# martende/findex

Hardware: AMD Instinct MI355X
Metric: rank_queries_per_sec (higher is better)
Workload: dtype u64

## Files before the change

### findex_amd/csrc/fmx_search4.h

```cpp
#pragma once
#include <type_traits>
#include "fmx_device.h"
#include "fmx_pool_deal.h"

namespace fmx {

constexpr int kSThreads = 256;

__device__ __forceinline__ uint32_t fetch4(const uint8_t *__restrict__ pat, uint64_t pos) {
  if (pos >= 4) {
    uint32_t d;
    __builtin_memcpy(&d, pat + pos - 4, 4);
    return __builtin_bswap32(d);
  }
  uint32_t r = 0;
  for (uint32_t j = 0; j < (uint32_t)pos; j++) r |= (uint32_t)pat[pos - 1 - j] << (8 * j);
  return r;
}


__device__ __forceinline__ uint32_t pat_chunk(const uint8_t *__restrict__ pat, const uint64_t *__restrict__ own,
                                              uint64_t end, uint32_t len, uint32_t j) {
  const uint32_t have = len > 4u * j ? len - 4u * j : 0u;
  const uint64_t pos = end - 4ull * j;
// ... 32 lines not shown
#ifdef FMX_SEARCHLOG
  const unsigned long long sl_t0 = __builtin_amdgcn_s_memrealtime();
  unsigned long long sl_t1 = 0, sl_look = 0, sl_draw = 0;
  uint32_t sl_claim = 0, sl_last = 0;
  uint32_t sl_batches = 0, sl_claims = 0;
#endif
  if (threadIdx.x == 0 && blockIdx.x < kCensusBlocks) {
    counters[(size_t)kCounterSlots * kCounterStride + 2u * blockIdx.x] = __builtin_amdgcn_s_memrealtime();
    if (blockIdx.x == 0) counters[(size_t)kCounterSlots * kCounterStride + 2u * kCensusBlocks] = gridDim.x;
  }
  if (spin & 0xFFFFu) {
    const unsigned long long c0 = __builtin_amdgcn_s_memrealtime();
    while (__builtin_amdgcn_s_memrealtime() - c0 < (spin & 0xFFFFu)) __builtin_amdgcn_s_sleep(32);
  }
  const uint32_t wave = (blockIdx.x * kSThreads + threadIdx.x) >> 6;
  const uint32_t nwaves = gridDim.x * (kSThreads / 64);
  const uint32_t grp = (threadIdx.x & 63) / G;
  auto load_off_raw = [&](uint64_t bt, uint64_t &v0, uint64_t &v1) {
    const uint64_t pid = bt * P + grp;
    const uint64_t *p = po.at(pid < k ? pid : (uint64_t)k - 1);
    v0 = p[0];
    v1 = p[1];
  };
  static_assert(kSThreads == 256, "one thread per symbol fills the tables in LDS");
  __shared__ uint4 s_tab[256];
  __shared__ uint8_t s_dense[KT ? 256 : 4];
  __shared__ uint16_t s_slot[KT ? 256 : 4];
  uint64_t raw0a, raw0b, raw1a, raw1b;
  {
    const uint4 sym = ix.symtab()[threadIdx.x];
    uint8_t dn = 0;
    uint16_t sl = 0;
    if (KT) { dn = kdense[threadIdx.x]; sl = ix.slot[threadIdx.x]; }
    load_off_raw(wave, raw0a, raw0b);
    load_off_raw((uint64_t)wave + nwaves, raw1a, raw1b);
    if (KT) { s_dense[threadIdx.x] = dn; s_slot[threadIdx.x] = sl; }
    s_tab[threadIdx.x] = sym;
  }
  __syncthreads();
  const LaneConst lc = lane_const<G2 ? 4 : G>();
  const uint32_t t = G2 ? (threadIdx.x & 1u) : lc.t;
  const uint32_t lane_off = t * 16;
  uint32_t steps = 0, reqs = 0;
  struct Blk { uint4 a, b; };
  auto blk_load = [&](uint64_t vb, uint32_t b1, uint32_t upto) -> Blk {
    const uint64_t at = vb + lane_off + (uint64_t)b1 * kBlockBytes;
    Blk w;
    w.a = load_line16(at);
    w.b = make_uint4(0, 0, 0, 0);
    if constexpr (G2) {
      if (upto >= 192u) w.b = load_line16(at + 32);
    }
    return w;
  };
  auto blk_rank = [&](const Blk &w, uint32_t m1) -> uint64_t {
    if constexpr (G2) return rank_finish_g2<WIDE>(Blk2{w.a, w.b}, m1, t);
    else return rank_finish<WIDE>(w.a, m1, lc);
  };
  auto blk_bit = [&](const Blk &w, uint32_t m1) -> uint32_t {
    if constexpr (G2) return payload_bit_g2(Blk2{w.a, w.b}, m1, t);
    else return payload_bit(w.a, m1, lc);
  };
  constexpr uint32_t RB = 1u;
  auto gbc0 = [&](uint32_t v) -> uint32_t { if constexpr (G2) return pair_bcast<0>(v); else return group_bcast<G, 0>(v); };
  auto gbc1 = [&](uint32_t v) -> uint32_t { if constexpr (G2) return pair_bcast<1>(v); else return group_bcast<G, 1>(v); };
  const uint32_t nbatch = (k + P - 1) / P;
  constexpr bool kPool = G2 || RW != 0u;
  const uint32_t tix_area = kPool ? (spin >> 16) & 0xFFu : 0u;
  const bool miss_none = JT != 0u && (spin >> 31) != 0u;
  uint32_t nstatic = nbatch;
  if (tix_area) {
    const uint32_t rounds = nbatch / nwaves, held = (spin >> 24) & 0xFu;
    if (rounds >= held + 2u) nstatic = (rounds - held) * nwaves;
  }
  constexpr bool kStage = LAYOUT != kLayoutBytes;
  constexpr uint32_t kStageBytes = G2 ? 2048 : 1024, kStagePad = 16;
  __shared__ __attribute__((aligned(16))) uint32_t s_pat[kSThreads / 64][2][kStage ? (kStagePad + kStageBytes + 16) / 4 : 4];
  uint32_t par = 0;
  constexpr bool kFold = (JT && RW == 0u) || RW != 0u;
  constexpr uint32_t kParkCap = RW ? 128u : (G2 ? 96u : 64u);
  __shared__ uint64_t s_park_row[kFold ? kSThreads / 64 : 1][kFold ? kParkCap : 1];
  __shared__ uint32_t s_park_pid[kFold ? kSThreads / 64 : 1][kFold ? kParkCap : 1];
  __shared__ uint32_t s_park_it[kFold ? kSThreads / 64 : 1][kFold ? kParkCap : 1];
  uint32_t npark = 0;
  constexpr uint32_t kRowsCap = 64u + P;
  __shared__ uint64_t s_rows_row[RW ? kSThreads / 64 : 1][RW ? kRowsCap : 1];
  __shared__ uint64_t s_rows_end[RW ? kSThreads / 64 : 1][RW ? kRowsCap : 1];
  __shared__ uint32_t s_rows_pid[RW ? kSThreads / 64 : 1][RW ? kRowsCap : 1];
  __shared__ uint32_t s_rows_it[RW ? kSThreads / 64 : 1][RW ? kRowsCap : 1];
  __shared__ uint32_t s_rows_len[RW ? kSThreads / 64 : 1][RW ? kRowsCap : 1];
  uint32_t nrows = 0;
  uint32_t rsteps = 0, rlooks = 0;
  auto st_out = [](auto *p, uint64_t v) { __builtin_nontemporal_store((decltype(*p + 0))v, p); };
  auto emit = [&](uint32_t q, uint64_t a, uint64_t b) {
    if (pk_cap != ~0ull) {
      unsigned long long *pk = reinterpret_cast<unsigned long long *>(sp_out);
      const uint64_t w = b - a;
      if (w >= kPackWide) {
        const unsigned long long slot = atomicAdd(pk + k, 1ull);
        if (slot < pk_cap) { pk[(uint64_t)k + 1 + 2 * slot] = q; pk[(uint64_t)k + 2 + 2 * slot] = b; }
      }
      st_out(pk + q, a | ((w < kPackWide ? w : kPackWide) << 40));
    } else {
      st_out(sp_out + q, a);
      st_out(ep_out + q, b);
    }
  };
  const uint32_t wave_in_wg = (uint32_t)__builtin_amdgcn_readfirstlane((int)(threadIdx.x >> 6));
  const uint32_t lane64 = threadIdx.x & 63u;
  const uint64_t pat_addr = (uint64_t)(uintptr_t)pat;
  auto fix_off = [&](uint64_t bt, uint64_t v0, uint64_t v1, uint64_t &e, uint32_t &len) {
    const uint64_t pid = bt * P + grp;
    const uint64_t q = pid < k ? pid : (uint64_t)k - 1;
    const uint64_t b = po.fixed ? q * po.fixed : v0;
    e = po.fixed ? (q + 1) * po.fixed : v1;
    len = pid < k ? (uint32_t)(e - b) : 0u;
  };
  struct Stage { uint4 w; uint4 w2; uint64_t base; bool ok; };
  auto stage_issue = [&](uint64_t e, uint32_t len) {
    const uint64_t b = e - len;
    const uint64_t b0 = ((uint64_t)__builtin_amdgcn_readfirstlane((int)(uint32_t)(b >> 32)) << 32) | (uint32_t)__builtin_amdgcn_readfirstlane((int)(uint32_t)b);
    const uint64_t e1 = ((uint64_t)(uint32_t)__builtin_amdgcn_readlane((int)(uint32_t)(e >> 32), 63) << 32) | (uint32_t)__builtin_amdgcn_readlane((int)(uint32_t)e, 63);
    Stage st;
    const uint64_t al = (pat_addr + b0) & ~15ull;
    const uint64_t span = pat_addr + e1 - al;
    st.ok = kStage && span <= kStageBytes;
    st.base = al - pat_addr;
    st.w = make_uint4(0, 0, 0, 0);
    if (st.ok && 16ull * lane64 < span) st.w = load_line16(al + 16u * lane64);
    st.w2 = make_uint4(0, 0, 0, 0);
    if constexpr (G2) {
      if (st.ok && 1024ull + 16ull * lane64 < span) st.w2 = load_line16(al + 1024u + 16u * lane64);
    }
    return st;
  };
  auto stage_park = [&](const Stage &st, uint32_t area) {
    if (st.ok) *reinterpret_cast<uint4 *>(s_pat[wave_in_wg][area] + (kStagePad + 16u * lane64) / 4) = st.w;
    if constexpr (G2) {
      if (st.ok) *reinterpret_cast<uint4 *>(s_pat[wave_in_wg][area] + (kStagePad + 1024u + 16u * lane64) / 4) = st.w2;
    }
  };
  constexpr uint32_t NT = KT ? KT / 4 : 1;
  struct Tail { uint32_t c[NT]; };
  uint64_t end0, end1, raw2a, raw2b;
  uint32_t len0, len1;
  uint32_t ktl = 0, jtl = 0, r3l = 0;
  fix_off(wave, raw0a, raw0b, end0, len0);
  fix_off((uint64_t)wave + nwaves, raw1a, raw1b, end1, len1);
  Stage cur = stage_issue(end0, len0);
  stage_park(cur, par);
  Tail tail_ahead;
#pragma unroll
  for (uint32_t i = 0; i < NT; i++) tail_ahead.c[i] = (!kStage && len0 > 4u * i) ? fetch4(pat, end0 - 4ull * i) : 0u;
  auto walk_step = [&](uint32_t c, uint64_t &wsp, uint64_t &wep) {
    const uint4 en = s_tab[c];
    const uint64_t cfc = ((uint64_t)en.y << 32) | en.x;
    const uint64_t vb = ((uint64_t)en.w << 32) | en.z;
    if (vb > 1) {
      if (LAYOUT == kLayoutBytes) {
        const ByteRankReq q1 = byte_rank_issue(ix, (uint16_t)(vb - 2), wsp, lc);
        wsp = cfc + byte_rank_finish(q1, c, lc);
        wep = wsp + byte_match_bit(q1, c, lc);
      } else {
        uint32_t b1, m1;
        split448(wsp, b1, m1);
        const Blk w1 = blk_load(vb, b1, m1);
        wsp = cfc + blk_rank(w1, m1);
        wep = wsp + blk_bit(w1, m1);
      }
      reqs += R * RB;
    } else {
      const uint64_t r1 = cfc + ((vb == 1 && wsp > ix.eof) ? 1u : 0u);
      wep = cfc + ((vb == 1 && wep > ix.eof) ? 1u : 0u);
      wsp = r1;
    }
    steps++;
  };
  auto walk_parked = [&](auto last_tag) {
    constexpr bool kLast = decltype(last_tag)::value;
    while (npark) {
      const uint32_t take = npark < P ? npark : P;
      const bool actw = grp < take;
      const uint32_t slot = npark - take + (actw ? grp : 0u);
      npark -= take;
      const uint32_t wpid = actw ? s_park_pid[wave_in_wg][slot] : 0u;
      uint32_t wit = actw ? s_park_it[wave_in_wg][slot] : 0u;
      uint64_t wsp = actw ? s_park_row[wave_in_wg][slot] : 0ull;
      uint32_t wj = (uint32_t)(wsp >> 56);
      const bool wnone = wj == 0xFFu;
      const bool wkx = KX && actw && wj == 0xFEu;
      wj = (wnone || wkx) ? 0u : wj;
      wsp &= (1ull << 56) - 1;
      if constexpr (R3T && kLast) {
        while (__builtin_amdgcn_ballot_w64(actw && wj >= 3u)) {
          const bool go = actw && wj >= 3u;
          if (go) {
            wsp = r3tab[wsp] & ((1ull << 40) - 1);
            wj -= 3u;
            wit += 3u;
            steps += 3u;
          }
          r3l += (uint32_t)__builtin_popcountll(__builtin_amdgcn_ballot_w64(go && t == 0));
        }
      }
      uint64_t wep = wsp + ((actw && !wnone && !wkx) ? 1u : 0u);
      uint64_t wbegin = 0, wend = 0;
      if (actw) po.get(wpid, wbegin, wend);
      const uint32_t wlen = (uint32_t)(wend - wbegin);
      if constexpr (KX) {
        if (__builtin_amdgcn_ballot_w64(wkx)) {
          uint32_t code = 0;
#pragma unroll
          for (uint32_t j = 0; j < KT; j++) code = code * ksigma + s_dense[wkx ? pat[wend - 1 - j] : 0u];
          const uint4 xe = ktab[wkx ? code : 0u];
          if (wkx) {
            const uint64_t xsp = (((uint64_t)xe.y << 32) | xe.x) & ((1ull << 56) - 1), xep = ((uint64_t)xe.w << 32) | xe.z;
            if (xsp < xep) {
              steps += KT + 1u;
            } else {
              wsp = xsp;
              wep = xep;
              steps += xe.y >> 24;
            }
          }
          ktl += (uint32_t)__builtin_popcountll(__builtin_amdgcn_ballot_w64(wkx && t == 0));
        }
      }
      for (;;) {
        const uint32_t wrem = wlen - wit;
        if (!__builtin_amdgcn_ballot_w64(actw && wsp < wep && wrem != 0u)) break;
        const uint32_t nst = wrem < 8u ? wrem : 8u;
        uint64_t chars = 0;
        if (actw && wsp < wep) {
          if (nst == 8u) {
            uint32_t lo, hi;
            __builtin_memcpy(&lo, pat + (wend - wit - 8), 4);
            __builtin_memcpy(&hi, pat + (wend - wit - 4), 4);
            chars = ((uint64_t)__builtin_bswap32(lo) << 32) | __builtin_bswap32(hi);
          } else {
            for (uint32_t s8 = 0; s8 < nst; s8++) chars |= (uint64_t)pat[wend - wit - 1 - s8] << (8u * s8);
          }
        }
        for (uint32_t s8 = 0; s8 < 8; s8++) {
          const bool stepping = actw && wsp < wep && s8 < nst;
          if (!__builtin_amdgcn_ballot_w64(stepping)) break;
          if (stepping) walk_step((uint32_t)(chars >> (8u * s8)) & 0xFFu, wsp, wep);
        }
        wit += nst;
      }
      if (actw && t == 0) emit(wpid, wsp, wep);
    }
  };
  auto rows_phase = [&](const bool all) {
    if constexpr (RW != 0u) {
      while (nrows >= (all ? 1u : 64u)) {
        const uint32_t take = nrows < 64u ? nrows : 64u;
        const bool on = lane64 < take;
        const uint32_t slot = nrows - take + (on ? lane64 : 0u);
        nrows -= take;
        uint64_t row = on ? s_rows_row[wave_in_wg][slot] : 0ull;
        const uint64_t rend = on ? s_rows_end[wave_in_wg][slot] : 0ull;
        const uint32_t rpid = on ? s_rows_pid[wave_in_wg][slot] : 0u;
        const uint32_t rlen = on ? s_rows_len[wave_in_wg][slot] : 0u;
        uint32_t rit = on ? s_rows_it[wave_in_wg][slot] : 0u;
        bool live = on;
        while (__builtin_amdgcn_ballot_w64(live)) {
          const uint32_t rem = rlen - rit;
          bool fail = false;
          if constexpr (RW == 3u) {
            const bool tm = live && rem >= 3u;
            unsigned long long re = 0;
            uint32_t d = 0;
            if (tm) {
              re = r3tab[row];
              __builtin_memcpy(&d, pat + (rend - rit - 3), 4);
            }
            if (tm && (uint32_t)(re >> 40) == __builtin_bswap32(d << 8)) {
              rlooks++;
              row = re & ((1ull << 40) - 1);
              rit += 3;
              rsteps += 3;
            } else if (live) {
              rlooks += tm ? 1u : 0u;
              if (rem == 0u) emit(rpid, row, row + 1);
              else fail = true;
              live = false;
            }
          } else {
            const bool rm = live && rem != 0u;
            unsigned long long re = 0;
            uint32_t c = 0;
            if (rm) {
              re = r3tab[row];
              c = pat[rend - rit - 1];
            }
            const uint32_t c2 = (uint32_t)(re >> 40) & 0xFFu;
            if (rm && c == c2 && c2 != 0u) {
              rlooks++;
              row = re & ((1ull << 40) - 1);
              rit++;
              rsteps++;
            } else if (live) {
              rlooks += rm ? 1u : 0u;
              if (rem == 0u) emit(rpid, row, row + 1);
              else fail = true;
              live = false;
            }
          }
          const unsigned long long fm = __builtin_amdgcn_ballot_w64(fail);
          if (fm) {
            const uint32_t ps = npark + (uint32_t)__builtin_popcountll(fm & ((1ull << lane64) - 1ull));
            if (fail) { s_park_row[wave_in_wg][ps] = row; s_park_pid[wave_in_wg][ps] = rpid; s_park_it[wave_in_wg][ps] = rit; }
            npark += (uint32_t)__builtin_popcountll(fm);
          }
        }
      }
    }
  };
  constexpr bool kLaneWalk = !(WIDE && JT == 1u && R3T && !G2);
  auto walk_last = [&]() {
    while (npark) {
      const uint32_t take = npark < 64u ? npark : 64u;
      const bool on = lane64 < take;
      const uint32_t slot = npark - take + (on ? lane64 : 0u);
      npark -= take;
      const uint32_t wpid = on ? s_park_pid[wave_in_wg][slot] : 0u;
      const uint32_t wit0 = on ? s_park_it[wave_in_wg][slot] : 0u;
      uint64_t wsp = on ? s_park_row[wave_in_wg][slot] : 0ull;
      uint32_t wj = (uint32_t)(wsp >> 56);
      const bool wnone = wj == 0xFFu;
      const bool wkx = KX && on && wj == 0xFEu;
      wj = (wnone || wkx) ? 0u : wj;
      wsp &= (1ull << 56) - 1;
      const uint32_t n3 = R3T ? wj / 3u : 0u;
      unsigned long long word = 0;
      if constexpr (R3T) word = r3tab[n3 >= 1u ? wsp : 0ull];
      const uint64_t *own = po.at(wpid);
      const uint64_t o0 = own[0], o1 = own[1];
      const uint32_t wit = wit0 + 3u * n3;
      rsteps += 3u * n3;
      if constexpr (R3T) {
        r3l += (uint32_t)__builtin_popcountll(__builtin_amdgcn_ballot_w64(n3 >= 1u)) + (uint32_t)__builtin_popcountll(__builtin_amdgcn_ballot_w64(n3 >= 2u));
        if (n3 >= 1u) wsp = word & ((1ull << 40) - 1);
        word = r3tab[n3 >= 2u ? wsp : 0ull];
      }
      const uint64_t wbegin = po.fixed ? (uint64_t)wpid * po.fixed : o0, wend = po.fixed ? ((uint64_t)wpid + 1) * po.fixed : o1;
      const uint32_t wlen = (uint32_t)(wend - wbegin);
      const uint32_t wrem = (on && !wnone && !wkx) ? wlen - wit : 0u;
      const uint32_t nst = wrem < 8u ? wrem : 8u;
      uint64_t chars = 0;
      {
        const uint8_t *src = (nst != 0u && wlen >= 8u) ? pat + (wend - wit - nst) : reinterpret_cast<const uint8_t *>(own);
        uint32_t lo, hi;
        __builtin_memcpy(&lo, src, 4);
        __builtin_memcpy(&hi, src + 4, 4);
        const uint64_t v = ((uint64_t)__builtin_bswap32(lo) << 32) | __builtin_bswap32(hi);
        if (nst != 0u && wlen >= 8u) chars = v >> (8u * (8u - nst));
      }
      uint64_t wep = wsp;
      if constexpr (KX) {
        uint32_t code = 0;
#pragma unroll
        for (uint32_t i = 0; i < KT / 4u; i++) {
          uint32_t d;
          __builtin_memcpy(&d, wkx ? pat + (wend - 4u * (i + 1u)) : reinterpret_cast<const uint8_t *>(own), 4);
          d = __builtin_bswap32(d);
#pragma unroll
          for (uint32_t j = 0; j < 4u; j++) code = code * ksigma + s_dense[(d >> (8u * j)) & 0xFFu];
        }
        const uint4 xe = ktab[wkx ? code : 0u];
        ktl += (uint32_t)__builtin_popcountll(__builtin_amdgcn_ballot_w64(wkx));
        if (wkx) {
          const uint64_t xsp = (((uint64_t)xe.y << 32) | xe.x) & ((1ull << 56) - 1), xep = ((uint64_t)xe.w << 32) | xe.z;
          if (xsp < xep) {
            rsteps += KT + 1u;
          } else {
            wsp = xsp;
            wep = xep;
            rsteps += xe.y >> 24;
          }
        }
      }
      if constexpr (R3T) {
        if (n3 >= 2u) wsp = word & ((1ull << 40) - 1);
        for (uint32_t lv = 3u; __builtin_amdgcn_ballot_w64(n3 >= lv); lv++) {
          if (n3 >= lv) wsp = r3tab[wsp] & ((1ull << 40) - 1);
          r3l += (uint32_t)__builtin_popcountll(__builtin_amdgcn_ballot_w64(n3 >= lv));
        }
      }
      if (on && nst != 0u && wlen < 8u) {
        for (uint32_t s8 = 0; s8 < nst; s8++) chars |= (uint64_t)pat[wend - wit - 1 - s8] << (8u * s8);
      }
      const bool walks = nst != 0u;
      if (on && !walks) emit(wpid, wsp, (wnone || wkx) ? wep : wsp + 1u);
      if (walks) {
        s_park_row[wave_in_wg][slot] = wsp | ((uint64_t)(nst | (nst == wrem ? 16u : 0u)) << 56);
        s_park_it[wave_in_wg][slot] = wit;
      }
      const unsigned long long wm = __builtin_amdgcn_ballot_w64(walks);
      const uint32_t slot0 = npark;
      for (uint32_t base = 0; base < take; base += P) {
        if (((wm >> base) & ((1ull << P) - 1ull)) == 0ull) continue;
        const bool actw = ((wm >> (base + grp)) & 1ull) != 0ull;
        const uint32_t gslot = slot0 + base + (actw ? grp : 0u);
        const uint64_t grow = s_park_row[wave_in_wg][gslot];
        const uint32_t gpid = s_park_pid[wave_in_wg][gslot], git = s_park_it[wave_in_wg][gslot];
        const uint32_t gnst = actw ? (uint32_t)(grow >> 56) & 15u : 0u;
        const bool gfinal = ((uint32_t)(grow >> 60) & 1u) != 0u;
        const int from = (int)(base + grp);
        const uint64_t gchars = ((uint64_t)(uint32_t)__shfl((int)(uint32_t)(chars >> 32), from, 64) << 32) | (uint32_t)__shfl((int)(uint32_t)chars, from, 64);
        uint64_t gsp = grow & ((1ull << 56) - 1);
        uint64_t gep = gsp + 1u;
        for (uint32_t s8 = 0; s8 < 8; s8++) {
          const bool stepping = actw && gsp < gep && s8 < gnst;
          if (!__builtin_amdgcn_ballot_w64(stepping)) break;
          if (stepping) walk_step((uint32_t)(gchars >> (8u * s8)) & 0xFFu, gsp, gep);
        }
        const bool again = actw && gsp < gep && !gfinal;
        if (actw && !again && t == 0) emit(gpid, gsp, gep);
        const unsigned long long am = __builtin_amdgcn_ballot_w64(again && t == 0);
        if (am) {
          const uint32_t ps = npark + (uint32_t)__builtin_popcountll(am & ((1ull << lane64) - 1ull));
          if (again && t == 0) { s_park_row[wave_in_wg][ps] = gsp; s_park_pid[wave_in_wg][ps] = gpid; s_park_it[wave_in_wg][ps] = git + gnst; }
          npark += (uint32_t)__builtin_popcountll(am);
        }
      }
    }
  };
#ifdef FMX_SEARCHLOG
  sl_t1 = __builtin_amdgcn_s_memrealtime();
#endif
  uint32_t batch = wave;
  Stage nxt_stage;
  {
    constexpr bool kClaimBeside = kPool && JT != 0u;
    [[maybe_unused]] unsigned long long *tix = nullptr;
    [[maybe_unused]] uint32_t drawn = 0;
    [[maybe_unused]] bool claimed = false;
    auto search_one_batch = [&](auto staged_tag, auto ahead_tag) {
    constexpr bool STAGED = decltype(staged_tag)::value;
    constexpr bool AHEAD = decltype(ahead_tag)::value;
    const uint32_t pid = batch * P + grp;
    const bool act = pid < k;
    const uint64_t *own = po.at(act ? pid : 0u);
    const uint64_t end = end0;
    const uint32_t len = act ? len0 : 0u;
    const uint64_t cur_base = cur.base;
    const uint32_t *const spat = s_pat[wave_in_wg][par];
    auto chunk = [&](uint32_t j) -> uint32_t {
      if constexpr (!STAGED) {
        return pat_chunk(pat, own, end, len, j);
      } else {
        const uint32_t have = len > 4u * j ? len - 4u * j : 0u;
        const uint32_t o = have ? (uint32_t)(end - 4ull * j - cur_base) + (kStagePad - 4u) : 0u;
        const uint32_t lo = spat[o >> 2], hi = spat[(o >> 2) + 1];
        const uint32_t r = __builtin_bswap32(__builtin_amdgcn_alignbyte(hi, lo, o & 3u));
        return have >= 4u ? r : (r & ((1u << (8u * have)) - 1u));
      }
    };
    auto chars4 = [&](uint32_t at) -> uint32_t {
      const uint32_t have = len > at ? len - at : 0u;
      if constexpr (STAGED) {
        const uint32_t o = have ? (uint32_t)(end - at - cur_base) + (kStagePad - 4u) : 0u;
        const uint32_t lo = spat[o >> 2], hi = spat[(o >> 2) + 1];
        const uint32_t r = __builtin_bswap32(__builtin_amdgcn_alignbyte(hi, lo, o & 3u));
        return have >= 4u ? r : (r & ((1u << (8u * have)) - 1u));
      } else {
        uint32_t r = 0;
        if (have >= 4u) {
          uint32_t d;
          __builtin_memcpy(&d, pat + (end - at - 4), 4);
          r = __builtin_bswap32(d);
        } else {
          for (uint32_t j = 0; j < have; j++) r |= (uint32_t)pat[end - at - 1 - j] << (8u * j);
        }
        return r;
      }
    };
    Tail tailq;
#pragma unroll
    for (uint32_t i = 0; i < NT; i++) {
      if constexpr (STAGED) tailq.c[i] = chunk(i);
      else if constexpr (kStage) tailq.c[i] = len > 4u * i ? fetch4(pat, end - 4ull * i) : 0u;
      else tailq.c[i] = act ? tail_ahead.c[i] : 0u;
    }
    uint32_t ch = tailq.c[0];
    uint32_t nx = chunk(KT ? KT / 4 + 1 : 1);
    auto issue_ahead = [&]() {
      if constexpr (AHEAD) {
        nxt_stage = stage_issue(end1, len1);
        if constexpr (!kStage) {
#pragma unroll
          for (uint32_t i = 0; i < NT; i++) tail_ahead.c[i] = len1 > 4u * i ? fetch4(pat, end1 - 4ull * i) : 0u;
        }
        load_off_raw((uint64_t)batch + 2ull * nwaves, raw2a, raw2b);
      }
    };
    if (KT == 0) { issue_ahead(); if constexpr (AHEAD) stage_park(nxt_stage, par ^ 1u); }
    uint64_t sp = 0, ep = ix.n;
    bool kx_parked = false;
    auto special = [&](uint64_t cfc, uint64_t vb, uint64_t x) { return cfc + ((vb == 1 && x > ix.eof) ? 1u : 0u); };
    if (KT == 0) {
      if (len > 0) {
        const uint32_t c = ch & 0xFFu;
        const uint4 e = s_tab[c];
        const uint4 e2 = s_tab[(c + 1) & 0xFFu];
// ... 4 lines not shown
        ep = vb > 1 ? nxt : special(cfc, vb, ix.n);
        steps++;
      }
      ch >>= 8;
    } else {
      uint32_t code = 0;
      bool elig = act && len >= KT;
#pragma unroll
      for (uint32_t j = 0; j < KT; j++) {
        const uint32_t d = s_dense[(tailq.c[j >> 2] >> (8u * (j & 3u))) & 0xFFu];
        elig = elig && d != 0xFFu;
        code = code * ksigma + d;
      }
      bool ex = false;
      uint32_t chk = 0;
      uint32_t zcode = 0;
      if constexpr (KX) {
        chk = chunk(KT / 4);
        bool ez = elig && len > KT;
#pragma unroll
        for (uint32_t j = 1; j <= KT; j++) {
          const uint32_t d = s_dense[((j < KT ? tailq.c[j < KT ? j >> 2 : 0u] : chk) >> (8u * (j & 3u))) & 0xFFu];
          ez = ez && d != 0xFFu;
          zcode = zcode * ksigma + d;
        }
        ex = ez;
      }
      const uint4 *ksrc = ktab + (elig ? code : 0u);
      if constexpr (KX) { if (ex) ksrc = kext + 2ull * zcode + (t & 1u); }
#ifdef FMX_SEARCHLOG
      if (!sl_look) sl_look = __builtin_amdgcn_s_memrealtime();
#endif
      const uint4 ent = *ksrc;
      issue_ahead();
      if (elig && !ex) {
        sp = (((uint64_t)ent.y << 32) | ent.x) & ((1ull << 56) - 1);
        ep = ((uint64_t)ent.w << 32) | ent.z;
        steps += ent.y >> 24;
      }
      ktl += (uint32_t)__builtin_popcountll(__builtin_amdgcn_ballot_w64(elig && t == 0));
      if constexpr (AHEAD) stage_park(nxt_stage, par ^ 1u);
      if constexpr (KX) {
        if (__builtin_amdgcn_ballot_w64(ex)) {
          const uint32_t half = t & 1u, y = tailq.c[0] & 0xFFu;
          const uint32_t h1 = gbc0(ent.y);
          const bool big = ((h1 >> 8) & 0xFFu) == 0xFFu;
          uint32_t lt = 0, le = 0;
          auto count16 = [&](const uint4 &w, uint32_t from) {
#pragma unroll
            for (uint32_t b = 0; b < 16; b++) {
              const uint32_t x = ((b < 4 ? w.x : b < 8 ? w.y : b < 12 ? w.z : w.w) >> (8u * (b & 3u))) & 0xFFu;
              lt += (b >= from && x < y) ? 1u : 0u;
              le += (b >= from && x <= y) ? 1u : 0u;
            }
          };
          if (ex && !big) count16(ent, half ? 0u : 6u);
          uint32_t cnt = (h1 >> 8) & 0xFFu;
          if (__builtin_amdgcn_ballot_w64(ex && big)) {
            const uint32_t h2 = gbc0(ent.z), h3 = gbc0(ent.w);
            const uint64_t off = (h1 >> 16) | ((uint64_t)(h2 & 0xFFFFFFu) << 16);
            const uint32_t bc = (h2 >> 24) | (h3 << 8);
            if (ex && big) cnt = bc;
            for (uint32_t i = 0;; i++) {
              const bool more = ex && big && 32u * i < bc;
              if (!__builtin_amdgcn_ballot_w64(more)) break;
              uint4 w = make_uint4(~0u, ~0u, ~0u, ~0u);
              if (more && 32u * i + 16u * half < bc) w = kovf[off + 2u * i + half];
              if (more) count16(w, 0u);
              ktl += (uint32_t)__builtin_popcountll(__builtin_amdgcn_ballot_w64(more && t == 0));
            }
          }
          lt = gbc0(lt) + gbc1(lt);
          le = y == 255u ? cnt : gbc0(le) + gbc1(le);
          const uint64_t spz = gbc0(ent.x) | ((uint64_t)(h1 & 0xFFu) << 32);
          if (ex) {
            sp = spz + lt;
            ep = spz + le;
          }
          const bool kxp = ex && sp >= ep;
          const unsigned long long pm = __builtin_amdgcn_ballot_w64(kxp && t == 0);
          if (pm) {
            const uint32_t slot = npark + (uint32_t)__builtin_popcountll(pm & ((1ull << lane64) - 1ull));
            if (kxp && t == 0) { s_park_row[wave_in_wg][slot] = sp | (0xFEull << 56); s_park_pid[wave_in_wg][slot] = pid; s_park_it[wave_in_wg][slot] = KT + 1u; }
            npark += (uint32_t)__builtin_popcountll(pm);
          }
          kx_parked = kxp;
          if (ex && !kxp) steps += KT + 1u;
        }
      }
      constexpr uint32_t kWalk = KX ? KT + 1u : KT;
      if (__builtin_amdgcn_ballot_w64(act && !(KX ? ex : elig))) {
        for (uint32_t j = 0; j < kWalk; j++) {
          const bool stepping = act && (KX ? (!ex && j >= (elig ? KT : 0u)) : !elig) && j < len && sp < ep;
          if (!__builtin_amdgcn_ballot_w64(stepping)) {
            if (KX && j < KT) continue;
            break;
          }
          if (stepping) {
            const uint32_t c = ((j < KT ? tailq.c[j < KT ? j >> 2 : 0u] : chk) >> (8u * (j & 3u))) & 0xFFu;
            const uint4 e = s_tab[c];
            if constexpr (G2) {
              const uint64_t cfc = ((uint64_t)e.y << 32) | e.x, vb = ((uint64_t)e.w << 32) | e.z;
              if (vb > 1) {
                uint32_t b1, b2, m1, m2;
                split448(sp, b1, m1);
                split448(ep, b2, m2);
                const Blk w1 = blk_load(vb, b1, b2 != b1 ? m1 : (m1 > m2 ? m1 : m2));
                Blk w2 = w1;
                if (b2 != b1) { w2 = blk_load(vb, b2, m2); reqs += RB; }
                sp = cfc + blk_rank(w1, m1);
                ep = cfc + blk_rank(w2, m2);
                reqs += RB;
              } else {
                const uint64_t r1 = cfc + ((vb == 1 && sp > ix.eof) ? 1u : 0u);
                ep = cfc + ((vb == 1 && ep > ix.eof) ? 1u : 0u);
                sp = r1;
              }
            } else {
              reqs += backward_step<WIDE, LAYOUT>(ix, c, s_slot[c], ((uint64_t)e.y << 32) | e.x, lc, sp, ep);
            }
            steps++;
          }
        }
      }
      if constexpr (KX) ch = chk >> 8;
      else ch = chunk(KT / 4);
    }
    constexpr uint32_t kIt0 = KX ? KT + 1u : (KT ? KT : 1u);
    uint32_t skip = 0;
    uint32_t cursor_it = kIt0;
    bool deferred = kx_parked;
    for (uint32_t it = kIt0;; it++) {
      bool alive = it < len && sp < ep;
      if constexpr (RW != 0u) {
        const bool hand = alive && (ep - sp) == 1 && (RW == 1u || (len - it) % RW == 0u);
        const unsigned long long hm = __builtin_amdgcn_ballot_w64(hand && t == 0);
        if (hm) {
          const uint32_t slot = nrows + (uint32_t)__builtin_popcountll(hm & ((1ull << lane64) - 1ull));
          if (hand && t == 0) {
            s_rows_row[wave_in_wg][slot] = sp; s_rows_end[wave_in_wg][slot] = end; s_rows_pid[wave_in_wg][slot] = pid;
            s_rows_it[wave_in_wg][slot] = it; s_rows_len[wave_in_wg][slot] = len;
          }
          nrows += (uint32_t)__builtin_popcountll(hm);
        }
        if (hand) {
          deferred = true;
          ep = sp;
          alive = false;
        }
      }
      if (!__builtin_amdgcn_ballot_w64(alive)) break;
      auto cursor_to = [&](uint32_t ni) {
        const uint32_t c0 = chars4(ni), a = ni & 3u;
        ch = a ? (c0 & ((1u << (8u * (4u - a))) - 1u)) : c0;
        nx = chunk((ni >> 2) + 1);
        cursor_it = ni;
      };
      auto chars12 = [&](uint32_t at, bool want, uint32_t &q0, uint32_t &q1, uint32_t &q2) {
        if constexpr (STAGED) {
          const uint32_t o = want ? (uint32_t)(end - at - cur_base) + (kStagePad - 12u) : 0u;
          const uint32_t w0 = o >> 2, sh = o & 3u;
          const uint32_t d0 = spat[w0], d1 = spat[w0 + 1], d2 = spat[w0 + 2], d3 = spat[w0 + 3];
          q0 = __builtin_bswap32(__builtin_amdgcn_alignbyte(d3, d2, sh));
          q1 = __builtin_bswap32(__builtin_amdgcn_alignbyte(d2, d1, sh));
          q2 = __builtin_bswap32(__builtin_amdgcn_alignbyte(d1, d0, sh));
        } else {
// ... 83 lines not shown
            const bool hit = mine && (d0 | d1 | d2) == 0u;
            missj = d0 ? (uint32_t)__builtin_ctz(d0) >> 3 : (d1 ? 4u + ((uint32_t)__builtin_ctz(d1) >> 3) : 8u + ((uint32_t)__builtin_ctz(d2 | 0x80000000u) >> 3));
            const uint32_t hm = (uint32_t)(__builtin_amdgcn_ballot_w64(hit) >> gbase) & ((1u << G) - 1u);
            const int first = (int)(gbase + (hm ? (uint32_t)__builtin_ctz(hm) : 0u));
            const uint32_t rlo = (uint32_t)__shfl((int)((je.z >> 24) | (je.w << 8)), first, 64), rhi = (uint32_t)__shfl((int)(je.w >> 24), first, 64);
            jumped = can && hm != 0u;
            rowj = ((uint64_t)rhi << 32) | rlo;
            nrows = (uint32_t)__builtin_popcount(hm);
            jtl += (uint32_t)__builtin_popcountll(__builtin_amdgcn_ballot_w64(mine));
            }
          }
          if (can) {
            if (!jumped && width == 1u) {
              park_now = true;
              deferred = true;
            }
            const uint32_t took = jumped ? (pair_both ? 2u * jc : jc) : 0u;
            if (pair_then_miss) { park_now = true; deferred = true; park_ahead = jc; }
            ep = (jumped && !pair_then_miss) ? rowj + nrows : ((deferred && !pair_then_miss) ? sp : (pair_then_miss ? rowj : ep));
            sp = jumped ? rowj : sp;
            steps += took;
            skip = pair_then_miss ? 0u : took;
            lookedup = jumped;
          }
        }
      }
      if (JT && R3T) {
        const uint64_t width = ep - sp;
        const bool want3 = alive && skip == 0u && !deferred && !lookedup && width >= 1u && width <= (uint64_t)RG && rem >= 3u &&
                           (rem < jc || it % 3u == 0u);
        if (__builtin_amdgcn_ballot_w64(want3)) {
          const uint32_t three = chars4(it) & 0xFFFFFFu;
          const uint32_t lane64 = threadIdx.x & 63u, base = lane64 - t;
          unsigned long long re = 0;
          uint32_t hm, lo3, hi3;
          bool mine;
          if constexpr (G2) {
            mine = want3 && (uint64_t)t < width;
            const bool mine1 = want3 && (uint64_t)(2u + t) < width;
            unsigned long long re1 = 0;
            if (mine) re = r3tab[sp + t];
            if (mine1) re1 = r3tab[sp + 2u + t];
            const bool h0 = mine && (uint32_t)(re >> 40) == three, h1 = mine1 && (uint32_t)(re1 >> 40) == three;
            hm = ((uint32_t)(__builtin_amdgcn_ballot_w64(h0) >> base) & 3u) | (((uint32_t)(__builtin_amdgcn_ballot_w64(h1) >> base) & 3u) << 2);
            const uint32_t fr = hm ? (uint32_t)__builtin_ctz(hm) : 0u;
            const unsigned long long rs = (fr >> 1) ? re1 : re;
            const int first = (int)(base + (fr & 1u));
            lo3 = (uint32_t)__shfl((int)(uint32_t)rs, first, 64);
            hi3 = (uint32_t)__shfl((int)(uint32_t)(rs >> 32), first, 64);
            r3l += (uint32_t)__builtin_popcountll(__builtin_amdgcn_ballot_w64(mine1));
          } else {
          mine = want3 && (uint64_t)t < width;
          if (mine) re = r3tab[sp + t];
          const bool hit = mine && (uint32_t)(re >> 40) == three;
          hm = (uint32_t)(__builtin_amdgcn_ballot_w64(hit) >> base) & ((1u << G) - 1u);
          const int first = (int)(base + (hm ? (uint32_t)__builtin_ctz(hm) : 0u));
          lo3 = (uint32_t)__shfl((int)(uint32_t)re, first, 64);
          hi3 = (uint32_t)__shfl((int)(uint32_t)(re >> 32), first, 64);
          }
          if (want3) {
            const bool took = hm != 0u;
            if (took) {
              sp = (((uint64_t)hi3 << 32) | lo3) & ((1ull << 40) - 1);
              ep = sp + (uint32_t)__builtin_popcount(hm);
              steps += 3;
              skip = 3u;
              lookedup = true;
            } else if (width == 1u) {
              park_now = true;
              deferred = true;
              ep = sp;
              missj = (uint32_t)__builtin_ctz((((uint32_t)(re >> 40) ^ three) & 0xFFFFFFu) | 0x80000000u) >> 3;
            }
          }
          r3l += (uint32_t)__builtin_popcountll(__builtin_amdgcn_ballot_w64(mine));
        }
      }
      if (JT && __builtin_amdgcn_ballot_w64(park_now)) {
        if constexpr (kFold) {
          if (miss_none && park_now) steps += missj + 1u;
          const unsigned long long pm = __builtin_amdgcn_ballot_w64(park_now && t == 0);
          const uint32_t lane64p = threadIdx.x & 63u;
          const uint32_t slot = npark + (uint32_t)__builtin_popcountll(pm & ((1ull << lane64p) - 1ull));
          if (park_now && t == 0) { s_park_row[wave_in_wg][slot] = miss_none ? (0xFFull << 56) : (sp | ((uint64_t)missj << 56)); s_park_pid[wave_in_wg][slot] = pid; s_park_it[wave_in_wg][slot] = it + park_ahead; }
          npark += (uint32_t)__builtin_popcountll(pm);
        }
      }
      if ((JT || R3T) && !__builtin_amdgcn_ballot_w64(alive && skip == 0u && !deferred)) {
        bool cand = alive && !deferred && skip != 0u;
        uint32_t adv = 0;
#pragma unroll
        for (int bit = (JT == 2u ? 4 : 3); bit >= 0; bit--) {
          const bool z = cand && ((skip >> bit) & 1u) == 0u;
          if (__builtin_amdgcn_ballot_w64(z)) cand = z;
          else adv |= 1u << bit;
        }
        if (!__builtin_amdgcn_ballot_w64(cand)) adv = 1u;
        skip -= skip >= adv ? adv : skip;
        it += adv - 1u;
        continue;
      }
      if constexpr (JT || R3T) {
        if (cursor_it != it) cursor_to(it);
      }
      const bool stepping = alive && skip == 0u && !deferred;
      skip -= skip ? 1u : 0u;
      const bool wide_iv = stepping && (ep - sp) != 1;
      if (!__builtin_amdgcn_ballot_w64(wide_iv)) {
        if (stepping) {
          const uint32_t c = ch & 0xFFu;
          const uint4 e = s_tab[c];
          const uint64_t cfc = ((uint64_t)e.y << 32) | e.x;
          const uint64_t vb = ((uint64_t)e.w << 32) | e.z;
          if (vb > 1) {
            if (LAYOUT == kLayoutBytes) {
              const ByteRankReq q1 = byte_rank_issue(ix, (uint16_t)(vb - 2), sp, lc);
              sp = cfc + byte_rank_finish(q1, c, lc);
              ep = sp + byte_match_bit(q1, c, lc);
            } else {
              uint32_t b1, m1;
              split448(sp, b1, m1);
              const Blk w1 = blk_load(vb, b1, m1);
              sp = cfc + blk_rank(w1, m1);
              ep = sp + blk_bit(w1, m1);
            }
            reqs += R * RB;
          } else {
            const uint64_t r1 = special(cfc, vb, sp);
            ep = special(cfc, vb, ep);
            sp = r1;
          }
          steps++;
        }
      } else if (stepping) {
        const uint32_t c = ch & 0xFFu;
        const uint4 e = s_tab[c];
        const uint64_t cfc = ((uint64_t)e.y << 32) | e.x;
        const uint64_t vb = ((uint64_t)e.w << 32) | e.z;
        if (vb > 1) {
          if (LAYOUT == kLayoutBytes) {
            const ByteRankReq q1 = byte_rank_issue(ix, (uint16_t)(vb - 2), sp, lc);
            ByteRankReq q2 = q1;
            const bool two = (ep >> 7) != (sp >> 7);
            if (two) q2 = byte_rank_issue(ix, (uint16_t)(vb - 2), ep, lc);
            else q2.rem = (uint32_t)ep & 127u;
            sp = cfc + byte_rank_finish(q1, c, lc);
            ep = cfc + byte_rank_finish(q2, c, lc);
            reqs += two ? 2 * R : R;
          } else {
            uint32_t b1, b2, m1, m2;
            split448(sp, b1, m1);
            split448(ep, b2, m2);
            const Blk w1 = blk_load(vb, b1, b2 != b1 ? m1 : (m1 > m2 ? m1 : m2));
            Blk w2 = w1;
            if (b2 != b1) { w2 = blk_load(vb, b2, m2); reqs += RB; }
            sp = cfc + blk_rank(w1, m1);
            ep = cfc + blk_rank(w2, m2);
            reqs += RB;
          }
        } else {
          const uint64_t r1 = special(cfc, vb, sp);
          ep = special(cfc, vb, ep);
          sp = r1;
        }
        steps++;
      }
      ch >>= 8;
      if ((it & 3u) == 3u) {
        ch = nx;
        nx = chunk((it >> 2) + 2);
      }
      cursor_it = it + 1u;
    }
    if (act && t == 0 && !deferred) emit(pid, sp, ep);
    };
    auto one_batch = [&](auto ahead_tag) {
      if constexpr (kStage) {
        if (cur.ok) search_one_batch(std::true_type{}, ahead_tag);
        else search_one_batch(std::false_type{}, ahead_tag);
      } else {
        search_one_batch(std::false_type{}, ahead_tag);
      }
      if constexpr (!decltype(ahead_tag)::value && kClaimBeside) {
        if (!claimed) {
          if (lane64 == 0) drawn = (uint32_t)atomicAdd(tix, 1ull);
#ifdef FMX_SEARCHLOG
          sl_claim = (uint32_t)(__builtin_amdgcn_s_memrealtime() - sl_t0);
          sl_claims += 1u << 16;
#endif
        }
      }
      if constexpr (RW != 0u) {
        if (nrows >= 64u) {
          if (npark > kParkCap - 64u) walk_parked(std::false_type{});
          rows_phase(false);
        }
      } else {
        if (kFold && npark > kParkCap - P) walk_parked(std::false_type{});
      }
    };
    for (; batch < nstatic; batch += nwaves) {
#ifdef FMX_SEARCHLOG
      sl_batches++;
#endif
      one_batch(std::true_type{});
      cur = nxt_stage;
      par ^= 1u;
      end0 = end1; len0 = len1;
      fix_off((uint64_t)batch + 2ull * nwaves, raw2a, raw2b, end1, len1);
    }
    if constexpr (kPool) {
    if (nstatic != nbatch) {
      static_assert(kPoolShards == kTixShards, "fmx_pool_deal.h deals to the counters of a ticket area");
      const uint32_t shard = pool_shard_of((uint32_t)__builtin_amdgcn_readfirstlane((int)wave), nwaves);
      tix = counters + (kCounterBytes + kCensusBytes + kCalibScratchBytes) / 8 +
            ((size_t)(tix_area - 1u) * kTixShards + shard) * kTixStride;
#ifdef FMX_SEARCHLOG
      sl_draw = __builtin_amdgcn_s_memrealtime();
      sl_claim = (uint32_t)(sl_draw - sl_t0);
#endif
      if (lane64 == 0) drawn = (uint32_t)atomicAdd(tix, 1ull);
      uint32_t ndraw = nwaves;
      asm volatile("" : "+s"(ndraw));
      const PoolDeal deal = pool_deal(ndraw, shard, nbatch - nstatic);
      const uint32_t first = nstatic + deal.first, pool = deal.count, last_draw = deal.count + deal.drawers - 1u;
      for (;;) {
        const uint32_t tk = (uint32_t)__builtin_amdgcn_readfirstlane((int)drawn);
        if (tk >= pool) {
          if (tk == last_draw && lane64 == 0) atomicExch(tix, 0ull);
          break;
        }
#ifdef FMX_SEARCHLOG
        sl_batches++;
        sl_last = sl_claim;
#endif
        if constexpr (!kClaimBeside) {
          if (lane64 == 0) drawn = (uint32_t)atomicAdd(tix, 1ull);
#ifdef FMX_SEARCHLOG
          sl_claim = (uint32_t)(__builtin_amdgcn_s_memrealtime() - sl_t0);
#endif
        }
        claimed = false;
        batch = first + tk;
        {
          uint64_t a0, a1;
          load_off_raw(batch, a0, a1);
          fix_off(batch, a0, a1, end0, len0);
        }
        cur = stage_issue(end0, len0);
        stage_park(cur, par);
#pragma unroll
        for (uint32_t i = 0; i < NT; i++) tail_ahead.c[i] = (!kStage && len0 > 4u * i) ? fetch4(pat, end0 - 4ull * i) : 0u;
        one_batch(std::false_type{});
      }
    }
    }
  }
  if constexpr (RW != 0u) {
    if (npark > kParkCap - 64u) walk_parked(std::false_type{});
    rows_phase(true);
  }
#ifdef FMX_SEARCHLOG
  const unsigned long long sl_tw = __builtin_amdgcn_s_memrealtime();
#endif
  if constexpr (kFold) {
    if constexpr (kLaneWalk) walk_last();
    else walk_parked(std::true_type{});
  }
#ifdef FMX_SEARCHLOG
  const unsigned long long sl_t2 = __builtin_amdgcn_s_memrealtime();
#endif
  counters_add(counters, (t == 0 ? 2ull * steps : 0ull) + 2ull * rsteps, (t == 0 ? steps : 0u) + rsteps, t == 0 ? reqs : 0u);
  if (RW) {
    const unsigned long long rl = wave_sum((unsigned long long)rlooks);
    if ((threadIdx.x & 63u) == 0 && rl) atomicAdd(counters + (size_t)(blockIdx.x % kCounterSlots) * kCounterStride + 11, rl);
  }
#ifdef FMX_SEARCHLOG
  if ((threadIdx.x & 63u) == 0 && wave < (1u << 15)) {
    unsigned long long *e = g_searchlog[wave];
    e[0] = sl_t0; e[1] = ((sl_t1 - sl_t0) & 0xFFFFFFFFull) | ((sl_tw - sl_t0) << 32); e[2] = sl_t2; e[3] = __builtin_amdgcn_s_memrealtime() | ((unsigned long long)sl_batches << 48);
    e[4] = sl_look; e[5] = sl_draw;
    e[6] = sl_last ? sl_t0 + sl_last : 0ull; e[7] = (unsigned long long)(sl_claims & 0xFFFFu) | ((unsigned long long)(sl_claims >> 16) << 32);
  }
#endif
  if (threadIdx.x == 0 && blockIdx.x < kCensusBlocks)
    counters[(size_t)kCounterSlots * kCounterStride + 2u * blockIdx.x + 1u] = __builtin_amdgcn_s_memrealtime();
  if (KT) {
    const unsigned long long lookups = ktl;
    if ((threadIdx.x & 63u) == 0 && lookups)
      atomicAdd(counters + (size_t)(blockIdx.x % kCounterSlots) * kCounterStride + 9, lookups);
  }
  if (JT) {
    const unsigned long long lookups = jtl;
    if ((threadIdx.x & 63u) == 0 && lookups)
      atomicAdd(counters + (size_t)(blockIdx.x % kCounterSlots) * kCounterStride + 10, lookups);
  }
  if (JT && R3T) {
// ... 70 lines not shown
```

Before: 620,000.

## Carry next pattern chars in shared memory with parked rows to skip refetch

When a query is parked mid-walk, the next up-to-8 pattern characters (or the k-mer code) and a small count/final flag are stored alongside the parked row in a new shared array. The row is narrowed to 48 bits so the metadata fits above it. On resume, the parked walk and the row walk use the carried characters and skip reloading the pattern offsets and bytes from global memory. The ticket shard is also computed from block and wave index rather than a readfirstlane of the wave id. This adds shared-memory traffic and assumes rows fit in 48 bits.

New measurement: 626,800 (median of 6 runs). +1.1%, better.

```diff
diff --git a/findex_amd/csrc/fmx_search4.h b/findex_amd/csrc/fmx_search4.h
--- a/findex_amd/csrc/fmx_search4.h
+++ b/findex_amd/csrc/fmx_search4.h
@@ -138,6 +138,10 @@
   __shared__ uint64_t s_park_row[kFold ? kSThreads / 64 : 1][kFold ? kParkCap : 1];
   __shared__ uint32_t s_park_pid[kFold ? kSThreads / 64 : 1][kFold ? kParkCap : 1];
   __shared__ uint32_t s_park_it[kFold ? kSThreads / 64 : 1][kFold ? kParkCap : 1];
+  constexpr bool kCarry = JT != 0u && RW == 0u && !(KX && !G2);
+  __shared__ uint64_t s_park_chr[kCarry ? kSThreads / 64 : 1][kCarry ? kParkCap : 1];
+  constexpr uint32_t kNotCarried = 0xFFu;
+  constexpr uint64_t kRowMask = kCarry ? (1ull << 48) - 1 : (1ull << 56) - 1;
   uint32_t npark = 0;
   constexpr uint32_t kRowsCap = 64u + P;
   __shared__ uint64_t s_rows_row[RW ? kSThreads / 64 : 1][RW ? kRowsCap : 1];
@@ -245,8 +249,16 @@
       uint32_t wj = (uint32_t)(wsp >> 56);
       const bool wnone = wj == 0xFFu;
       const bool wkx = KX && actw && wj == 0xFEu;
+      uint32_t wmeta = kNotCarried;
+      uint64_t wchr = 0;
+      if constexpr (kCarry) {
+        wmeta = actw ? (uint32_t)(wsp >> 48) & 0xFFu : kNotCarried;
+        wchr = actw ? s_park_chr[wave_in_wg][slot] : 0ull;
+        if (R3T && !kLast && wj >= 3u && wj < 0xFEu) wmeta = kNotCarried;
+      }
+      bool carried = kCarry && wmeta != kNotCarried && !wnone && !wkx;
       wj = (wnone || wkx) ? 0u : wj;
-      wsp &= (1ull << 56) - 1;
+      wsp &= kRowMask;
       if constexpr (R3T && kLast) {
         while (__builtin_amdgcn_ballot_w64(actw && wj >= 3u)) {
           const bool go = actw && wj >= 3u;
@@ -261,13 +273,15 @@
       }
       uint64_t wep = wsp + ((actw && !wnone && !wkx) ? 1u : 0u);
       uint64_t wbegin = 0, wend = 0;
-      if (actw) po.get(wpid, wbegin, wend);
-      const uint32_t wlen = (uint32_t)(wend - wbegin);
+      if (actw && !(kCarry && (carried || wnone || wkx))) po.get(wpid, wbegin, wend);
+      uint32_t wlen = carried ? wit + (wmeta & 15u) : (uint32_t)(wend - wbegin);
       if constexpr (KX) {
         if (__builtin_amdgcn_ballot_w64(wkx)) {
-          uint32_t code = 0;
+          uint32_t code = (uint32_t)wchr;
+          if constexpr (!kCarry) {
 #pragma unroll
-          for (uint32_t j = 0; j < KT; j++) code = code * ksigma + s_dense[wkx ? pat[wend - 1 - j] : 0u];
+            for (uint32_t j = 0; j < KT; j++) code = code * ksigma + s_dense[wkx ? pat[wend - 1 - j] : 0u];
+          }
           const uint4 xe = ktab[wkx ? code : 0u];
           if (wkx) {
             const uint64_t xsp = (((uint64_t)xe.y << 32) | xe.x) & ((1ull << 56) - 1), xep = ((uint64_t)xe.w << 32) | xe.z;
@@ -287,7 +301,9 @@
         if (!__builtin_amdgcn_ballot_w64(actw && wsp < wep && wrem != 0u)) break;
         const uint32_t nst = wrem < 8u ? wrem : 8u;
         uint64_t chars = 0;
-        if (actw && wsp < wep) {
+        if (carried) {
+          chars = wchr;
+        } else if (actw && wsp < wep) {
           if (nst == 8u) {
             uint32_t lo, hi;
             __builtin_memcpy(&lo, pat + (wend - wit - 8), 4);
@@ -303,6 +319,13 @@
           if (stepping) walk_step((uint32_t)(chars >> (8u * s8)) & 0xFFu, wsp, wep);
         }
         wit += nst;
+        if constexpr (kCarry) {
+          if (carried && wsp < wep && (wmeta & 16u) == 0u) {
+            po.get(wpid, wbegin, wend);
+            wlen = (uint32_t)(wend - wbegin);
+          }
+          carried = false;
+        }
       }
       if (actw && t == 0) emit(wpid, wsp, wep);
     }
@@ -387,12 +410,20 @@
       const bool wnone = wj == 0xFFu;
       const bool wkx = KX && on && wj == 0xFEu;
       wj = (wnone || wkx) ? 0u : wj;
-      wsp &= (1ull << 56) - 1;
+      uint32_t wmeta = kNotCarried;
+      uint64_t wchr = 0;
+      if constexpr (kCarry) {
+        wmeta = on ? (uint32_t)(wsp >> 48) & 0xFFu : 0u;
+        wchr = on ? s_park_chr[wave_in_wg][slot] : 0ull;
+      }
+      wsp &= kRowMask;
+      const bool wmem = wmeta == kNotCarried;
       const uint32_t n3 = R3T ? wj / 3u : 0u;
       unsigned long long word = 0;
       if constexpr (R3T) word = r3tab[n3 >= 1u ? wsp : 0ull];
       const uint64_t *own = po.at(wpid);
-      const uint64_t o0 = own[0], o1 = own[1];
+      uint64_t o0 = 0, o1 = 0;
+      if (!kCarry || wmem) { o0 = own[0]; o1 = own[1]; }
       const uint32_t wit = wit0 + 3u * n3;
       rsteps += 3u * n3;
       if constexpr (R3T) {
@@ -402,10 +433,11 @@
       }
       const uint64_t wbegin = po.fixed ? (uint64_t)wpid * po.fixed : o0, wend = po.fixed ? ((uint64_t)wpid + 1) * po.fixed : o1;
       const uint32_t wlen = (uint32_t)(wend - wbegin);
-      const uint32_t wrem = (on && !wnone && !wkx) ? wlen - wit : 0u;
-      const uint32_t nst = wrem < 8u ? wrem : 8u;
+      const uint32_t wrem = (wmem && on && !wnone && !wkx) ? wlen - wit : 0u;
+      const uint32_t nst = wmem ? (wrem < 8u ? wrem : 8u) : (wmeta & 15u);
+      const bool wfinal = wmem ? nst == wrem : (wmeta & 16u) != 0u;
       uint64_t chars = 0;
-      {
+      if (!kCarry || wmem) {
         const uint8_t *src = (nst != 0u && wlen >= 8u) ? pat + (wend - wit - nst) : reinterpret_cast<const uint8_t *>(own);
         uint32_t lo, hi;
         __builtin_memcpy(&lo, src, 4);
@@ -413,16 +445,21 @@
         const uint64_t v = ((uint64_t)__builtin_bswap32(lo) << 32) | __builtin_bswap32(hi);
         if (nst != 0u && wlen >= 8u) chars = v >> (8u * (8u - nst));
       }
+      if constexpr (kCarry) {
+        if (!wmem) chars = wchr;
+      }
       uint64_t wep = wsp;
       if constexpr (KX) {
-        uint32_t code = 0;
+        uint32_t code = (uint32_t)wchr;
+        if constexpr (!kCarry) {
 #pragma unroll
-        for (uint32_t i = 0; i < KT / 4u; i++) {
-          uint32_t d;
-          __builtin_memcpy(&d, wkx ? pat + (wend - 4u * (i + 1u)) : reinterpret_cast<const uint8_t *>(own), 4);
-          d = __builtin_bswap32(d);
+          for (uint32_t i = 0; i < KT / 4u; i++) {
+            uint32_t d;
+            __builtin_memcpy(&d, wkx ? pat + (wend - 4u * (i + 1u)) : reinterpret_cast<const uint8_t *>(own), 4);
+            d = __builtin_bswap32(d);
 #pragma unroll
-          for (uint32_t j = 0; j < 4u; j++) code = code * ksigma + s_dense[(d >> (8u * j)) & 0xFFu];
+            for (uint32_t j = 0; j < 4u; j++) code = code * ksigma + s_dense[(d >> (8u * j)) & 0xFFu];
+          }
         }
         const uint4 xe = ktab[wkx ? code : 0u];
         ktl += (uint32_t)__builtin_popcountll(__builtin_amdgcn_ballot_w64(wkx));
@@ -444,13 +481,13 @@
           r3l += (uint32_t)__builtin_popcountll(__builtin_amdgcn_ballot_w64(n3 >= lv));
         }
       }
-      if (on && nst != 0u && wlen < 8u) {
+      if (wmem && on && nst != 0u && wlen < 8u) {
         for (uint32_t s8 = 0; s8 < nst; s8++) chars |= (uint64_t)pat[wend - wit - 1 - s8] << (8u * s8);
       }
       const bool walks = nst != 0u;
       if (on && !walks) emit(wpid, wsp, (wnone || wkx) ? wep : wsp + 1u);
       if (walks) {
-        s_park_row[wave_in_wg][slot] = wsp | ((uint64_t)(nst | (nst == wrem ? 16u : 0u)) << 56);
+        s_park_row[wave_in_wg][slot] = wsp | ((uint64_t)(nst | (wfinal ? 16u : 0u)) << 56);
         s_park_it[wave_in_wg][slot] = wit;
       }
       const unsigned long long wm = __builtin_amdgcn_ballot_w64(walks);
@@ -477,7 +514,7 @@
         const unsigned long long am = __builtin_amdgcn_ballot_w64(again && t == 0);
         if (am) {
           const uint32_t ps = npark + (uint32_t)__builtin_popcountll(am & ((1ull << lane64) - 1ull));
-          if (again && t == 0) { s_park_row[wave_in_wg][ps] = gsp; s_park_pid[wave_in_wg][ps] = gpid; s_park_it[wave_in_wg][ps] = git + gnst; }
+          if (again && t == 0) { s_park_row[wave_in_wg][ps] = gsp | (kCarry ? (uint64_t)kNotCarried << 48 : 0ull); s_park_pid[wave_in_wg][ps] = gpid; s_park_it[wave_in_wg][ps] = git + gnst; }
           npark += (uint32_t)__builtin_popcountll(am);
         }
       }
@@ -648,6 +685,9 @@
           if (pm) {
             const uint32_t slot = npark + (uint32_t)__builtin_popcountll(pm & ((1ull << lane64) - 1ull));
             if (kxp && t == 0) { s_park_row[wave_in_wg][slot] = sp | (0xFEull << 56); s_park_pid[wave_in_wg][slot] = pid; s_park_it[wave_in_wg][slot] = KT + 1u; }
+            if constexpr (kCarry) {
+              if (kxp && t == 0) s_park_chr[wave_in_wg][slot] = code;
+            }
             npark += (uint32_t)__builtin_popcountll(pm);
           }
           kx_parked = kxp;
@@ -897,7 +937,18 @@
           const unsigned long long pm = __builtin_amdgcn_ballot_w64(park_now && t == 0);
           const uint32_t lane64p = threadIdx.x & 63u;
           const uint32_t slot = npark + (uint32_t)__builtin_popcountll(pm & ((1ull << lane64p) - 1ull));
-          if (park_now && t == 0) { s_park_row[wave_in_wg][slot] = miss_none ? (0xFFull << 56) : (sp | ((uint64_t)missj << 56)); s_park_pid[wave_in_wg][slot] = pid; s_park_it[wave_in_wg][slot] = it + park_ahead; }
+          uint64_t cmeta = 0;
+          if constexpr (kCarry) {
+            cmeta = (uint64_t)kNotCarried << 48;
+            if constexpr (STAGED) {
+              const uint32_t cat = it + park_ahead + (R3T ? 3u * (missj / 3u) : 0u);
+              const uint32_t crem = park_now ? len - cat : 0u;
+              const uint64_t cchr = (uint64_t)chars4(cat) | ((uint64_t)chars4(cat + 4u) << 32);
+              cmeta = (uint64_t)((crem < 8u ? crem : 8u) | (crem <= 8u ? 16u : 0u)) << 48;
+              if (park_now && t == 0) s_park_chr[wave_in_wg][slot] = cchr;
+            }
+          }
+          if (park_now && t == 0) { s_park_row[wave_in_wg][slot] = miss_none ? (0xFFull << 56) : (sp | ((uint64_t)missj << 56) | cmeta); s_park_pid[wave_in_wg][slot] = pid; s_park_it[wave_in_wg][slot] = it + park_ahead; }
           npark += (uint32_t)__builtin_popcountll(pm);
         }
       }
@@ -1027,7 +1078,7 @@
     if constexpr (kPool) {
     if (nstatic != nbatch) {
       static_assert(kPoolShards == kTixShards, "fmx_pool_deal.h deals to the counters of a ticket area");
-      const uint32_t shard = pool_shard_of((uint32_t)__builtin_amdgcn_readfirstlane((int)wave), nwaves);
+      const uint32_t shard = pool_shard_of(blockIdx.x * (kSThreads / 64) + wave_in_wg, nwaves);
       tix = counters + (kCounterBytes + kCensusBytes + kCalibScratchBytes) / 8 +
             ((size_t)(tix_area - 1u) * kTixShards + shard) * kTixStride;
 #ifdef FMX_SEARCHLOG
```
